# MarcinKadziolka/nerf-sampling

Hardware: NVIDIA B200
Metric: rays_per_sec (higher is better)
Workload: dtype fp16 operands, fp32 accumulate (+ bf16 hi/lo split re-evaluation of the guard band)

## Files before the change

nerf_sampling_b200/csrc/mlp_fast.cuh:

```cuda
#pragma once
#include <type_traits>

#include "ptx.cuh"

namespace b200 {
namespace fast {

constexpr int TILE_M = 128;
constexpr int KC_STRIDE = 2048;
constexpr int ENC_KB = 16;
constexpr int VIEW_KB = 20;
constexpr int TILE_KC = 44;
constexpr int TILE_ACT_BYTES = TILE_KC * KC_STRIDE;
constexpr int RING_BYTES = 32768;
constexpr int AUX_FLOATS = 3080;
constexpr int SF32_FLOATS = 1032;
constexpr int SBIAS16 = 7 * 256;
constexpr int THREADS = 512;
constexpr int NSTEPS = 9;
constexpr int EPI_WARP0 = 4, EPI_WARPS = 8, PRO_WARP0 = 12, PRO_WARPS = 4;
constexpr size_t FOLD_BIAS_OFF = 65 * 16384;
constexpr size_t WPACK_BYTES = FOLD_BIAS_OFF + 512;

enum : uint32_t { AUX_B0 = 0, AUX_BF = 2048, AUX_BV = 2304, AUX_WA = 2432, AUX_BA = 2688, AUX_WR = 2692, AUX_BR = 3076 };
enum : uint32_t { SF_B7 = 0, SF_BV = 256, SF_WA = 384, SF_BA = 640, SF_WR = 644, SF_BR = 1028 };

__host__ __device__ constexpr int step_nk1(int s) { return s == 0 ? 4 : 16; }
__host__ __device__ constexpr int step_kb1(int s) { return s == 0 ? ENC_KB : 0; }
__host__ __device__ constexpr int step_nk2(int s) { return s == 5 ? 4 : (s == NSTEPS - 1 ? 2 : 0); }
__host__ __device__ constexpr int step_kb2(int s) { return s == 5 ? ENC_KB : VIEW_KB; }
__host__ __device__ constexpr int step_n(int s) { return s == NSTEPS - 1 ? 128 : 256; }
__host__ __device__ constexpr int step_nk(int s) { return step_nk1(s) + step_nk2(s); }
__host__ __device__ constexpr int step_stages(int s) { return s == NSTEPS - 1 ? 5 : step_nk(s) / 2; }
__host__ __device__ constexpr uint32_t step_woff(int s) {
  uint32_t o = 0;
  for (int i = 0; i < s; ++i) o += static_cast<uint32_t>(step_stages(i)) * 16384u;
  return o;
}

struct alignas(64) TMap {
  uint8_t bytes[128];
};

struct FastParams {
  const uint8_t* wpack;
  const float* aux;
  int n_rows;
  int S;
  const float* rays_o;
  const float* rays_d;
  const float* viewdirs;
  const float* z;
  const float* pts;
  float* out;
  int* guard_count;
  int* guard_list;
  int guard_cap;
  float guard_kappa;
  long long* timeline;
};

#ifdef B200NERF_TIMELINE
#define TL_STAMP(role, idx, j)                                                                         \
  do {                                                                                                 \
    if (p.timeline != nullptr && blockIdx.x == 0 && (idx) < 80) p.timeline[((role) * 80 + (idx)) * 4 + (j)] = clock64(); \
  } while (0)
#else
#define TL_STAMP(role, idx, j) \
  do {                         \
  } while (0)
#endif

constexpr int NSTAGE = 4;
constexpr int STAGE_BYTES = RING_BYTES / NSTAGE;
constexpr int NCTA = 2;
#ifndef B200NERF_FAST_STAGGER
#define B200NERF_FAST_STAGGER 5
#endif
constexpr int STAGGER = B200NERF_FAST_STAGGER;

struct __align__(16) Tail {
  uint64_t full[NSTAGE];
  uint64_t empty[NSTAGE];
  uint64_t acc_full[2];
  uint64_t a_ready[2];
  uint64_t enc_ready[2];
  uint64_t view_ready[2];
  uint64_t pts_free[2];
  uint64_t view_free[2];
  uint32_t tmem_base;
  uint32_t pad[3];
  float alpha_part[2][TILE_M];
  float eabs_part[2][TILE_M];
  float rgb_part[2][3][TILE_M];
};

__host__ __device__ constexpr int smem_bytes() {
  return 2 * TILE_ACT_BYTES + RING_BYTES + SF32_FLOATS * 4 + SBIAS16 * 2 + static_cast<int>(sizeof(Tail));
}

template <bool FP16>
__device__ __forceinline__ void store8(uint8_t* dst, const float (&v)[8]) {
  *reinterpret_cast<uint4*>(dst) = make_uint4(pack_half2<FP16, false>(v[0], v[1]), pack_half2<FP16, false>(v[2], v[3]),
                                              pack_half2<FP16, false>(v[4], v[5]), pack_half2<FP16, false>(v[6], v[7]));
}

template <bool FP16, int NF, int NCHUNK>
__device__ __forceinline__ void encode_store(const float (&x)[3], uint8_t* dst ) {
  float sn[NF][3], cs[NF][3];
#pragma unroll
  for (int t = 0; t < 3; ++t) {
    sincosf(x[t], &sn[0][t], &cs[0][t]);
    if (NF > 5) sincosf(x[t] * 32.0f, &sn[5][t], &cs[5][t]);
#pragma unroll
    for (int j = 1; j < NF; ++j) {
      if (j == 5) continue;
      const float s = sn[j - 1][t], c = cs[j - 1][t];
      sn[j][t] = 2.0f * s * c;
      cs[j][t] = (c - s) * (c + s);
    }
  }
  constexpr int NCOL = 3 + 6 * NF;
#pragma unroll
  for (int ch = 0; ch < NCHUNK; ++ch) {
    float v[8];
#pragma unroll
    for (int i = 0; i < 8; ++i) {
      const int cc = ch * 8 + i;
      if (cc < 3) v[i] = x[cc];
      else if (cc < NCOL) v[i] = ((cc - 3) % 6) < 3 ? sn[(cc - 3) / 6][(cc - 3) % 6] : cs[(cc - 3) / 6][(cc - 3) % 6 - 3];
      else v[i] = 0.f;
    }
    store8<FP16>(dst + ch * KC_STRIDE, v);
  }
}

template <bool FP16>
__device__ __noinline__ void encode_pts_lt10(int nf, float x0, float x1, float x2, uint8_t* dst) {
  const float x[3] = {x0, x1, x2};
  switch (nf) {
    case 1: encode_store<FP16, 1, 8>(x, dst); break;
    case 2: encode_store<FP16, 2, 8>(x, dst); break;
    case 3: encode_store<FP16, 3, 8>(x, dst); break;
    case 4: encode_store<FP16, 4, 8>(x, dst); break;
    case 5: encode_store<FP16, 5, 8>(x, dst); break;
    case 6: encode_store<FP16, 6, 8>(x, dst); break;
    case 7: encode_store<FP16, 7, 8>(x, dst); break;
    case 8: encode_store<FP16, 8, 8>(x, dst); break;
    default: encode_store<FP16, 9, 8>(x, dst); break;
  }
}
template <bool FP16>
__device__ __noinline__ void encode_view_lt4(int nv, float v0, float v1, float v2, uint8_t* dst) {
  const float v[3] = {v0, v1, v2};
  switch (nv) {
    case 1: encode_store<FP16, 1, 4>(v, dst); break;
    case 2: encode_store<FP16, 2, 4>(v, dst); break;
    default: encode_store<FP16, 3, 4>(v, dst); break;
  }
}
// ... 71 lines not shown
  epi_store32_packed<RELU, FP16>(va, bias16 + 64, dst + 8 * KC_STRIDE);
  tmem_ld_wait();
  epi_store32_packed<RELU, FP16>(vb, bias16 + 96, dst + 12 * KC_STRIDE);
}

template <int MODE, bool FP16>
__device__ __forceinline__ void epilogue_store(uint32_t tacc, const float* bias, const float* hw, uint8_t* dst,
                                               float& hsum, float& habs) {
  uint32_t va[32], vb[32];
  tmem_ld_32x32b_x32(tacc, va);
  tmem_ld_wait();
  tmem_ld_32x32b_x32(tacc + 32, vb);
  epi_store32<MODE, FP16>(va, bias, hw, dst, hsum, habs);
  tmem_ld_wait();
  tmem_ld_32x32b_x32(tacc + 64, va);
  epi_store32<MODE, FP16>(vb, bias + 32, hw + 32, dst + 4 * KC_STRIDE, hsum, habs);
  tmem_ld_wait();
  tmem_ld_32x32b_x32(tacc + 96, vb);
  epi_store32<MODE, FP16>(va, bias + 64, hw + 64, dst + 8 * KC_STRIDE, hsum, habs);
  tmem_ld_wait();
  epi_store32<MODE, FP16>(vb, bias + 96, hw + 96, dst + 12 * KC_STRIDE, hsum, habs);
}

__device__ __forceinline__ void epi_rgb32(const uint32_t (&v)[32], const float* bias, const float* wr, float& r, float& g,
                                          float& b) {
#pragma unroll
  for (int j = 0; j < 32; j += 4) {
    const float4 bb = *reinterpret_cast<const float4*>(bias + j);
    const float4 w0 = *reinterpret_cast<const float4*>(wr + j);
    const float4 w1 = *reinterpret_cast<const float4*>(wr + 128 + j);
    const float4 w2 = *reinterpret_cast<const float4*>(wr + 256 + j);
    const float x0 = fmaxf(__uint_as_float(v[j]) + bb.x, 0.f), x1 = fmaxf(__uint_as_float(v[j + 1]) + bb.y, 0.f);
    const float x2 = fmaxf(__uint_as_float(v[j + 2]) + bb.z, 0.f), x3 = fmaxf(__uint_as_float(v[j + 3]) + bb.w, 0.f);
    r = fmaf(x0, w0.x, r); r = fmaf(x1, w0.y, r); r = fmaf(x2, w0.z, r); r = fmaf(x3, w0.w, r);
    g = fmaf(x0, w1.x, g); g = fmaf(x1, w1.y, g); g = fmaf(x2, w1.z, g); g = fmaf(x3, w1.w, g);
    b = fmaf(x0, w2.x, b); b = fmaf(x1, w2.y, b); b = fmaf(x2, w2.z, b); b = fmaf(x3, w2.w, b);
  }
}

__device__ __forceinline__ bool input_is_finite(const FastParams& p, int grow) {
  const int ray = grow / p.S;
  float m = 0.f;
  if (p.pts != nullptr) {
#pragma unroll
    for (int t = 0; t < 3; ++t) m += fabsf(__ldg(p.pts + static_cast<size_t>(grow) * 3 + t));
  } else {
    const float zz = __ldg(p.z + grow);
#pragma unroll
    for (int t = 0; t < 3; ++t) m += fabsf(__fadd_rn(__ldg(p.rays_o + ray * 3 + t), __fmul_rn(__ldg(p.rays_d + ray * 3 + t), zz)));
  }
#pragma unroll
  for (int t = 0; t < 3; ++t) m += fabsf(__ldg(p.viewdirs + ray * 3 + t));
  return m < __int_as_float(0x7f800000);
}

template <bool FP16>
__global__ void __launch_bounds__(THREADS, 1)
nerf_fast_kernel(const __grid_constant__ FastParams p, const __grid_constant__ TMap tm_full) {
  extern __shared__ __align__(1024) uint8_t smem[];
  uint8_t* act = smem;
  uint8_t* ring = smem + 2 * TILE_ACT_BYTES;
  float* sf32 = reinterpret_cast<float*>(ring + RING_BYTES);
  uint16_t* sb16 = reinterpret_cast<uint16_t*>(ring + RING_BYTES + SF32_FLOATS * 4);
  Tail* tail = reinterpret_cast<Tail*>(ring + RING_BYTES + SF32_FLOATS * 4 + SBIAS16 * 2);

  const int warp = __shfl_sync(0xffffffffu, static_cast<int>(threadIdx.x >> 5), 0);
  const int lane = threadIdx.x & 31;
  const uint32_t rank = __shfl_sync(0xffffffffu, cluster_ctarank(), 0);
  const bool leader = rank == 0;
  const int cluster_id = blockIdx.x / NCTA;
  const int n_clusters = gridDim.x / NCTA;
  const int num_tiles = (p.n_rows + TILE_M - 1) / TILE_M;
  const int n_units = (num_tiles + 2 * NCTA - 1) / (2 * NCTA);
  const int my_units = cluster_id < n_units ? (n_units - cluster_id + n_clusters - 1) / n_clusters : 0;
  const int n_ticks = my_units > 0 ? my_units * NSTEPS + STAGGER : 0;

  if (threadIdx.x == 0) {
    for (int i = 0; i < NSTAGE; ++i) {
      mbar_init(&tail->full[i], 1);
      mbar_init(&tail->empty[i], 1);
    }
    for (int i = 0; i < 2; ++i) {
      mbar_init(&tail->acc_full[i], 1);
      mbar_init(&tail->a_ready[i], EPI_WARPS * NCTA);
      mbar_init(&tail->enc_ready[i], PRO_WARPS * NCTA);
      mbar_init(&tail->view_ready[i], PRO_WARPS * NCTA);
      mbar_init(&tail->pts_free[i], 1);
      mbar_init(&tail->view_free[i], 1);
    }
    fence_mbar_init();
  }
  if (warp == 2) {
    tmem_alloc_cg2(&tail->tmem_base, 512);
    tmem_relinquish_cg2();
  }
  for (int i = threadIdx.x; i < SF32_FLOATS; i += THREADS) {
    if (i >= 256 && i < 384) {
      sf32[i] = reinterpret_cast<const float*>(p.wpack + FOLD_BIAS_OFF)[i - 256];
    } else {
      const uint32_t src = i < 256 ? AUX_B0 + 7 * 256 + i : i < 640 ? AUX_WA + (i - 384)
                         : i < 644 ? AUX_BA + (i - 640) : i < 1028 ? AUX_WR + (i - 644) : AUX_BR + (i - 1028);
      sf32[i] = p.aux[src];
    }
  }
  for (int i = threadIdx.x; i < SBIAS16; i += THREADS) {
    sb16[i] = static_cast<uint16_t>(pack_half2<FP16, false>(p.aux[AUX_B0 + i], 0.f) & 0xffffu);
  }
  tc_fence_before();
  cluster_sync_all();
  tc_fence_after();
  const uint32_t tmem_base = __shfl_sync(0xffffffffu, tail->tmem_base, 0);
  const uint32_t tail_addr = smem_u32(tail);
  const uint32_t full_addr = tail_addr + offsetof(Tail, full), empty_addr = tail_addr + offsetof(Tail, empty);

  if (warp == 0) {
    if (lane == 0) tma_prefetch_desc(&tm_full);
    const uint32_t ring_addr = smem_u32(ring);
    const uint32_t lead_full = mapa_u32(full_addr, 0);
    uint32_t stage = 0, phase = 0;
    for (int i = 0; i < n_ticks; ++i) {
      for (int slot = 0; slot < 2; ++slot) {
        const int j = i - slot * STAGGER;
        if (j < 0 || j >= my_units * NSTEPS) continue;
        const int s = j % NSTEPS;
        const int n2 = step_stages(s);
        const int row0 = static_cast<int>((step_woff(s) + rank * static_cast<uint32_t>(n2) * STAGE_BYTES) / 512u);
        for (int k2 = 0; k2 < n2; ++k2) {
          mbar_wait_sleepy(empty_addr + stage * 8u, phase ^ 1u, 100);
          if (elect_one()) {
            if (leader) mbar_arrive_expect_tx_addr(full_addr + stage * 8u, 2u * STAGE_BYTES);
            tma_load_2d_cg2(ring_addr + stage * STAGE_BYTES, &tm_full, 0, row0 + k2 * (STAGE_BYTES / 512), lead_full + stage * 8u);
          }
          __syncwarp();
          if (++stage == NSTAGE) {
            stage = 0;
            phase ^= 1u;
          }
        }
      }
    }
  } else if (warp == 1) {
    if (leader) {
      const uint32_t act_addr = smem_u32(act);
      const uint32_t ring_addr = smem_u32(ring);
      const uint32_t acc_full_addr = tail_addr + offsetof(Tail, acc_full);
      const uint32_t a_ready_addr = tail_addr + offsetof(Tail, a_ready);
      const uint32_t enc_ready_addr = tail_addr + offsetof(Tail, enc_ready);
      const uint32_t view_ready_addr = tail_addr + offsetof(Tail, view_ready);
      const uint32_t pts_free_addr = tail_addr + offsetof(Tail, pts_free);
      const uint32_t view_free_addr = tail_addr + offsetof(Tail, view_free);
      constexpr uint32_t A_STEP = (2 * KC_STRIDE) >> 4;
      constexpr uint32_t DESC_HI = static_cast<uint32_t>(((128ull >> 4) << 32 | (1ull << 46)) >> 32);
      constexpr uint32_t A_LBO = (KC_STRIDE >> 4) << 16;
      uint32_t stage = 0, phase = 0, ca[2] = {0, 0}, ce[2] = {0, 0}, cv[2] = {0, 0};

      auto issue_stage = [&](auto acc_first, uint32_t d_tmem, uint32_t a_lo, uint32_t b_lbo, uint32_t piece16, uint32_t idesc) {
        mbar_wait_lean(full_addr + stage * 8u, phase);
        tc_fence_after();
        const uint32_t b_lo = b_lbo | ((ring_addr + stage * STAGE_BYTES) >> 4);
        if (elect_one()) {
          const uint64_t a0 = (static_cast<uint64_t>(DESC_HI) << 32) | a_lo;
          const uint64_t b0 = (static_cast<uint64_t>(DESC_HI) << 32) | b_lo;
          tc_mma_f16_cg2_imm<decltype(acc_first)::value>(d_tmem, a0, b0, idesc);
          tc_mma_f16_cg2_imm<true>(d_tmem, a0 + A_STEP, b0 + piece16, idesc);
          tc_commit_cg2_addr(empty_addr + stage * 8u, 3);
        }
        stage = (stage + 1) & (NSTAGE - 1);
        phase ^= (stage == 0);
      };

      auto issue_stage4 = [&](auto acc_first, auto two_only, uint32_t d_tmem, uint32_t a_lo, uint32_t a_lo2, uint32_t idesc) {
        constexpr uint32_t B_LBO = ((128u * 8u) >> 4) << 16, PIECE16 = 128;
        mbar_wait_lean(full_addr + stage * 8u, phase);
        tc_fence_after();
        const uint32_t b_lo = B_LBO | ((ring_addr + stage * STAGE_BYTES) >> 4);
        if (elect_one()) {
          const uint64_t a0 = (static_cast<uint64_t>(DESC_HI) << 32) | a_lo;
          const uint64_t a2 = (static_cast<uint64_t>(DESC_HI) << 32) | a_lo2;
          const uint64_t b0 = (static_cast<uint64_t>(DESC_HI) << 32) | b_lo;
          tc_mma_f16_cg2_imm<decltype(acc_first)::value>(d_tmem, a0, b0, idesc);
          tc_mma_f16_cg2_imm<true>(d_tmem, a0 + A_STEP, b0 + PIECE16, idesc);
          if (!decltype(two_only)::value) {
            tc_mma_f16_cg2_imm<true>(d_tmem, a2, b0 + 2 * PIECE16, idesc);
            tc_mma_f16_cg2_imm<true>(d_tmem, a2 + A_STEP, b0 + 3 * PIECE16, idesc);
          }
          tc_commit_cg2_addr(empty_addr + stage * 8u, 3);
        }
        stage = (stage + 1) & (NSTAGE - 1);
        phase ^= (stage == 0);
      };

#pragma unroll 1
      for (int i = 0; i < n_ticks; ++i) {
#pragma unroll
        for (int slot = 0; slot < 2; ++slot) {
          const int j = i - slot * STAGGER;
          if (j < 0 || j >= my_units * NSTEPS) continue;
          const int s = j % NSTEPS;
          const bool first = j < NSTEPS;
          const int n1 = step_nk1(s) / 2, n2 = step_nk(s) / 2;
          const uint32_t n = static_cast<uint32_t>(step_n(s));
          const uint32_t piece16 = n;
          const uint32_t idesc = umma_idesc_f16(FP16 ? 0u : 1u, 256, n);
          const uint32_t b_lbo = ((n * 8u) >> 4) << 16;
          const uint32_t kb1 = step_kb1(s), kb2 = step_kb2(s);
          [[maybe_unused]] const int tl_idx = j * 2 + slot;
          if (lane == 0) TL_STAMP(0, tl_idx, 0);
          if (s == 0) {
            mbar_wait_lean(enc_ready_addr + slot * 8u, ce[slot]++ & 1u);
            if (!first) mbar_wait_lean(a_ready_addr + slot * 8u, ca[slot]++ & 1u);
          } else {
            mbar_wait_lean(a_ready_addr + slot * 8u, ca[slot]++ & 1u);
          }
          if (s == NSTEPS - 1) mbar_wait_lean(view_ready_addr + slot * 8u, cv[slot]++ & 1u);
          if (lane == 0) TL_STAMP(0, tl_idx, 1);
          const uint32_t d_tmem = tmem_base + slot * 256u;
          const uint32_t a_base = A_LBO | ((act_addr + slot * TILE_ACT_BYTES) >> 4);
          uint32_t a_lo = a_base + kb1 * A_STEP;
          if (s == NSTEPS - 1) {
            issue_stage4(std::false_type{}, std::false_type{}, d_tmem, a_lo, a_lo + 2 * A_STEP, idesc);
#pragma unroll 1
            for (int k4 = 1; k4 < 4; ++k4) {
              a_lo += 4 * A_STEP;
              issue_stage4(std::true_type{}, std::false_type{}, d_tmem, a_lo, a_lo + 2 * A_STEP, idesc);
            }
            a_lo = a_base + VIEW_KB * A_STEP;
            issue_stage4(std::true_type{}, std::true_type{}, d_tmem, a_lo, a_lo, idesc);
          } else {
            issue_stage(std::false_type{}, d_tmem, a_lo, b_lbo, piece16, idesc);
            for (int k2 = 1; k2 < n1; ++k2) {
              a_lo += 2 * A_STEP;
              issue_stage(std::true_type{}, d_tmem, a_lo, b_lbo, piece16, idesc);
            }
            a_lo = a_base + kb2 * A_STEP;
            for (int k2 = n1; k2 < n2; ++k2) {
              issue_stage(std::true_type{}, d_tmem, a_lo, b_lbo, piece16, idesc);
              a_lo += 2 * A_STEP;
            }
          }
          if (elect_one()) {
            tc_commit_cg2_addr(acc_full_addr + slot * 8u, 3);
            if (s == 5) tc_commit_cg2_addr(pts_free_addr + slot * 8u, 3);
            if (s == NSTEPS - 1) tc_commit_cg2_addr(view_free_addr + slot * 8u, 3);
          }
          if (lane == 0) TL_STAMP(0, tl_idx, 2);
        }
      }
    }
  } else if (warp >= PRO_WARP0) {
    const int row = (warp - PRO_WARP0) * 32 + lane;
    const int row_off = (row >> 3) * 128 + (row & 7) * 16;
    const uint32_t pts_free_addr = tail_addr + offsetof(Tail, pts_free);
    const uint32_t view_free_addr = tail_addr + offsetof(Tail, view_free);
    const uint32_t enc_bar = mapa_u32(tail_addr + offsetof(Tail, enc_ready), 0);
    const uint32_t view_bar = mapa_u32(tail_addr + offsetof(Tail, view_ready), 0);
    const int nf = static_cast<int>(sf32[SF_BA + 1]), nv = static_cast<int>(sf32[SF_BA + 2]);
    const bool nf_full = nf == 0 || nf == 10, nv_full = nv == 0 || nv == 4;
    uint32_t cp[2] = {0, 0}, cw[2] = {0, 0};
    bool first = true;
    for (int u = cluster_id; u < n_units; u += n_clusters) {
#pragma unroll
      for (int slot = 0; slot < 2; ++slot) {
        const int grow = ((u * NCTA + static_cast<int>(rank)) * 2 + slot) * TILE_M + row;
        float x[3] = {0.f, 0.f, 0.f};
        if (grow < p.n_rows) {
          if (p.pts != nullptr) {
#pragma unroll
            for (int t = 0; t < 3; ++t) x[t] = __ldg(p.pts + static_cast<size_t>(grow) * 3 + t);
          } else {
            const int ray = grow / p.S;
            const float zz = __ldg(p.z + grow);
#pragma unroll
            for (int t = 0; t < 3; ++t)
              x[t] = __fadd_rn(__ldg(p.rays_o + ray * 3 + t), __fmul_rn(__ldg(p.rays_d + ray * 3 + t), zz));
          }
        }
        if (!first) {
          mbar_wait_sleepy(pts_free_addr + slot * 8u, cp[slot]++ & 1u, 500);
          tc_fence_after();
        }
        uint8_t* enc_dst = act + slot * TILE_ACT_BYTES + ENC_KB * 2 * KC_STRIDE + row_off;
        if (nf_full) encode_store<FP16, 10, 8>(x, enc_dst);
        else encode_pts_lt10<FP16>(nf, x[0], x[1], x[2], enc_dst);
        fence_proxy_async_smem();
        __syncwarp();
        if (lane == 0) mbar_arrive_remote(enc_bar + slot * 8u);
        float v[3] = {0.f, 0.f, 0.f};
        if (grow < p.n_rows) {
          const int ray = grow / p.S;
#pragma unroll
          for (int t = 0; t < 3; ++t) v[t] = __ldg(p.viewdirs + ray * 3 + t);
        }
        if (!first) {
          mbar_wait_sleepy(view_free_addr + slot * 8u, cw[slot]++ & 1u, 500);
          tc_fence_after();
        }
        uint8_t* view_dst = act + slot * TILE_ACT_BYTES + VIEW_KB * 2 * KC_STRIDE + row_off;
        if (nv_full) encode_store<FP16, 4, 4>(v, view_dst);
        else encode_view_lt4<FP16>(nv, v[0], v[1], v[2], view_dst);
        fence_proxy_async_smem();
        __syncwarp();
        if (lane == 0) mbar_arrive_remote(view_bar + slot * 8u);
      }
      first = false;
    }
  } else if (warp >= EPI_WARP0) {
    const int q = warp & 3;
    const int hf = (warp - EPI_WARP0) >> 2;
    const int row = q * 32 + lane;
    const int row_off = (row >> 3) * 128 + (row & 7) * 16;
    const uint32_t t_lane = tmem_base + (static_cast<uint32_t>(q * 32) << 16);
    const uint32_t acc_full_addr = tail_addr + offsetof(Tail, acc_full);
    const uint32_t rdy_bar = mapa_u32(tail_addr + offsetof(Tail, a_ready), 0);
    uint32_t cf[2] = {0, 0};
    float alpha_keep[2] = {0.f, 0.f}, eabs_keep[2] = {0.f, 0.f};

#pragma unroll 1
    for (int i = 0; i < n_ticks; ++i) {
      {
#pragma unroll
        for (int slot = 0; slot < 2; ++slot) {
          const int j = i - slot * STAGGER;
          if (j < 0 || j >= my_units * NSTEPS) continue;
          const int s = j % NSTEPS;
          const int u = cluster_id + (j / NSTEPS) * n_clusters;
          [[maybe_unused]] const int tl_idx = j * 2 + slot;
          if (lane == 0 && q == 0) TL_STAMP(1 + hf, tl_idx, 0);
          mbar_wait_lean(acc_full_addr + slot * 8u, cf[slot]++ & 1u);
          tc_fence_after();
          if (lane == 0 && q == 0) TL_STAMP(1 + hf, tl_idx, 1);
          const uint32_t tacc = t_lane + slot * 256u;
          uint8_t* a_tile = act + slot * TILE_ACT_BYTES;
          if (s < NSTEPS - 1) {
            uint8_t* dst = a_tile + hf * 16 * KC_STRIDE + row_off;
            if (s == 7) {
              float hs = 0.f, ha = 0.f;
              const int grow0 = ((u * NCTA + static_cast<int>(rank)) * 2 + slot) * TILE_M + (row & ~31);
              const bool need_abs = p.guard_count != nullptr && (p.S - 1 - grow0 % p.S) < 32;
              if (need_abs) epilogue_store<1, FP16>(tacc + hf * 128, sf32 + SF_B7 + hf * 128, sf32 + SF_WA + hf * 128, dst, hs, ha);
              else epilogue_store<3, FP16>(tacc + hf * 128, sf32 + SF_B7 + hf * 128, sf32 + SF_WA + hf * 128, dst, hs, ha);
              if (hf == 1) {
                tail->alpha_part[slot][row] = hs;
                tail->eabs_part[slot][row] = ha;
              } else {
                alpha_keep[slot] = hs;
                eabs_keep[slot] = ha;
              }
            } else {
              epilogue_store_packed<true, FP16>(tacc + hf * 128, sb16 + s * 256 + hf * 128, dst);
            }
          } else {
            float r = 0.f, g = 0.f, b = 0.f;
            uint32_t va[32], vb[32];
            tmem_ld_32x32b_x32(tacc + hf * 64, va);
            tmem_ld_wait();
            tmem_ld_32x32b_x32(tacc + hf * 64 + 32, vb);
            epi_rgb32(va, sf32 + SF_BV + hf * 64, sf32 + SF_WR + hf * 64, r, g, b);
            tmem_ld_wait();
            epi_rgb32(vb, sf32 + SF_BV + hf * 64 + 32, sf32 + SF_WR + hf * 64 + 32, r, g, b);
            if (hf == 1) {
              tail->rgb_part[slot][0][row] = r;
              tail->rgb_part[slot][1][row] = g;
              tail->rgb_part[slot][2][row] = b;
            }
            named_bar_sync(2 + q, 64);
            if (hf == 0) {
              r += tail->rgb_part[slot][0][row];
              g += tail->rgb_part[slot][1][row];
              b += tail->rgb_part[slot][2][row];
              const int grow = ((u * NCTA + static_cast<int>(rank)) * 2 + slot) * TILE_M + row;
              const bool valid = grow < p.n_rows;
              float sigma = alpha_keep[slot] + tail->alpha_part[slot][row] + sf32[SF_BA];
              if (valid) {
                if (!input_is_finite(p, grow)) r = g = b = sigma = __int_as_float(0x7fc00000);
                reinterpret_cast<float4*>(p.out)[grow] =
                    make_float4(r + sf32[SF_BR], g + sf32[SF_BR + 1], b + sf32[SF_BR + 2], sigma);
              }
              if (p.guard_count != nullptr) {
                const float eabs = eabs_keep[slot] + tail->eabs_part[slot][row] + fabsf(sf32[SF_BA]);
                const bool flag = valid && (grow % p.S) == p.S - 1 && !(fabsf(sigma) >= p.guard_kappa * eabs);
                const uint32_t m = __ballot_sync(0xffffffffu, flag);
                if (m != 0) {
                  int base = 0;
                  if (lane == 0) base = atomicAdd(p.guard_count, __popc(m));
                  base = __shfl_sync(0xffffffffu, base, 0);
                  const int idx = base + __popc(m & ((1u << lane) - 1u));
                  if (flag && idx < p.guard_cap) p.guard_list[idx] = grow;
                }
              }
            }
          }
          if (s < NSTEPS - 1) fence_proxy_async_smem();
          tc_fence_before();
          __syncwarp();
          if (lane == 0) mbar_arrive_remote(rdy_bar + slot * 8u);
          if (lane == 0 && q == 0) TL_STAMP(1 + hf, tl_idx, 2);
        }
      }
    }
  }

  __syncwarp();
  tc_fence_before();
  cluster_sync_all();
  if (warp == 2) tmem_dealloc_cg2(tmem_base, 512);
}

}
}
```

nerf_sampling_b200/csrc/ptx.cuh:

```cuda
#pragma once
#include <cstdint>
#include <cuda_runtime.h>

namespace b200 {

__device__ __forceinline__ uint32_t smem_u32(const void* p) {
  return static_cast<uint32_t>(__cvta_generic_to_shared(p));
}

__device__ __forceinline__ void mbar_init(uint64_t* bar, uint32_t count) {
  asm volatile("mbarrier.init.shared::cta.b64 [%0], %1;" ::"r"(smem_u32(bar)), "r"(count) : "memory");
}
__device__ __forceinline__ void fence_mbar_init() {
  asm volatile("fence.mbarrier_init.release.cluster;" ::: "memory");
}
__device__ __forceinline__ void mbar_arrive(uint64_t* bar) {
  asm volatile("mbarrier.arrive.shared::cta.b64 _, [%0];" ::"r"(smem_u32(bar)) : "memory");
}
__device__ __forceinline__ void mbar_arrive_expect_tx(uint64_t* bar, uint32_t bytes) {
  asm volatile("mbarrier.arrive.expect_tx.shared::cta.b64 _, [%0], %1;" ::"r"(smem_u32(bar)), "r"(bytes)
               : "memory");
}
__device__ __forceinline__ bool mbar_try_wait(uint64_t* bar, uint32_t parity) {
  uint32_t ok;
// ... 201 lines not shown
  uint32_t polls = 0;
  for (;;) {
    uint32_t ok;
    asm volatile(
        "{\n\t"
        ".reg .pred p;\n\t"
        "mbarrier.try_wait.parity.shared::cta.b64 p, [%1], %2;\n\t"
        "selp.u32 %0, 1, 0, p;\n\t"
        "}\n"
        : "=r"(ok)
        : "r"(bar_addr), "r"(parity)
        : "memory");
    if (ok) return;
    if (++polls > (1u << 24)) {
      printf("b200nerf: mbarrier wait timed out (block %d thread %d bar %u parity %u)\n", blockIdx.x, threadIdx.x, bar_addr, parity);
      __trap();
    }
  }
}
__device__ __forceinline__ void mbar_wait_sleepy(uint32_t bar_addr, uint32_t parity, uint32_t ns) {
  uint32_t polls = 0;
  for (;;) {
    uint32_t ok;
    asm volatile(
        "{\n\t"
        ".reg .pred p;\n\t"
        "mbarrier.try_wait.parity.shared::cta.b64 p, [%1], %2;\n\t"
        "selp.u32 %0, 1, 0, p;\n\t"
        "}\n"
        : "=r"(ok)
        : "r"(bar_addr), "r"(parity)
        : "memory");
    if (ok) return;
    __nanosleep(ns);
    if (++polls > (1u << 24)) {
      printf("b200nerf: mbarrier wait timed out (block %d thread %d bar %u parity %u)\n", blockIdx.x, threadIdx.x, bar_addr, parity);
      __trap();
    }
  }
}

__device__ __forceinline__ void mbar_arrive_remote(uint32_t cluster_addr) {
  asm volatile("mbarrier.arrive.shared::cluster.b64 _, [%0];" ::"r"(cluster_addr) : "memory");
}
__device__ __forceinline__ void mbar_arrive_expect_tx_addr(uint32_t bar_addr, uint32_t bytes) {
  asm volatile("mbarrier.arrive.expect_tx.shared::cta.b64 _, [%0], %1;" ::"r"(bar_addr), "r"(bytes) : "memory");
}
__device__ __forceinline__ bool elect_one() {
  uint32_t pred;
  asm volatile(
      "{\n\t"
      ".reg .pred p;\n\t"
      "elect.sync _|p, 0xffffffff;\n\t"
      "selp.u32 %0, 1, 0, p;\n\t"
      "}\n"
      : "=r"(pred));
  return pred != 0;
}
__device__ __forceinline__ void tc_commit_cg2_addr(uint32_t bar_addr, uint16_t cta_mask) {
  asm volatile("tcgen05.commit.cta_group::2.mbarrier::arrive::one.shared::cluster.multicast::cluster.b64 [%0], %1;" ::"r"(bar_addr),
               "h"(cta_mask)
               : "memory");
}
template <bool ACC>
__device__ __forceinline__ void tc_mma_f16_cg2_imm(uint32_t d_tmem, uint64_t a_desc, uint64_t b_desc, uint32_t idesc) {
  if (ACC) {
    asm volatile(
        "{\n\t.reg .pred p;\n\tsetp.eq.u32 p, 1, 1;\n\t"
        "tcgen05.mma.cta_group::2.kind::f16 [%0], %1, %2, %3, p;\n\t}\n" ::"r"(d_tmem),
        "l"(a_desc), "l"(b_desc), "r"(idesc)
        : "memory");
  } else {
    asm volatile(
        "{\n\t.reg .pred p;\n\tsetp.eq.u32 p, 1, 0;\n\t"
        "tcgen05.mma.cta_group::2.kind::f16 [%0], %1, %2, %3, p;\n\t}\n" ::"r"(d_tmem),
        "l"(a_desc), "l"(b_desc), "r"(idesc)
        : "memory");
  }
}

__device__ __forceinline__ void named_bar_sync(uint32_t id, uint32_t nthreads) {
  asm volatile("bar.sync %0, %1;" ::"r"(id), "r"(nthreads) : "memory");
}
__device__ __forceinline__ uint32_t pack_bf16x2(float lo_elem, float hi_elem) {
  uint32_t r;
  asm("cvt.rn.bf16x2.f32 %0, %1, %2;" : "=r"(r) : "f"(hi_elem), "f"(lo_elem));
  return r;
}

}
```

Measured before the change: 17.89 million.

## Give each accumulator slot its own epilogue warpgroup and rebalance registers with setmaxnreg

Raises the block from 512 to 768 threads so each of the two TMEM accumulator slots gets a dedicated set of 8 epilogue warps, instead of one set of epilogue warps alternating between both slots. This is meant to remove serialization between the two slots' epilogues so the MMA issuer waits less on a_ready. Control warps release registers via setmaxnreg.dec and worker warps claim more via setmaxnreg.inc, and the slot stagger is bumped from 5 to 6. The cost is lower per-thread register headroom, which risks spills, plus more warps contending for issue slots and shared memory.

```diff
diff --git a/nerf_sampling_b200/csrc/mlp_fast.cuh b/nerf_sampling_b200/csrc/mlp_fast.cuh
--- a/nerf_sampling_b200/csrc/mlp_fast.cuh
+++ b/nerf_sampling_b200/csrc/mlp_fast.cuh
@@ -16,9 +16,11 @@
 constexpr int AUX_FLOATS = 3080;
 constexpr int SF32_FLOATS = 1032;
 constexpr int SBIAS16 = 7 * 256;
-constexpr int THREADS = 512;
+constexpr int THREADS = 768;
 constexpr int NSTEPS = 9;
-constexpr int EPI_WARP0 = 4, EPI_WARPS = 8, PRO_WARP0 = 12, PRO_WARPS = 4;
+constexpr int EPI_WARP0 = 4, EPI_WARPS_PER_SLOT = 8, PRO_WARP0 = 20, PRO_WARPS = 4;
+constexpr int REG_CTRL = 40, REG_WORK = 88;
+static_assert(REG_CTRL + 5 * REG_WORK <= 6 * 80, "setmaxnreg budgets exceed the launch allocation");
 constexpr size_t FOLD_BIAS_OFF = 65 * 16384;
 constexpr size_t WPACK_BYTES = FOLD_BIAS_OFF + 512;
 
@@ -75,7 +77,7 @@
 constexpr int STAGE_BYTES = RING_BYTES / NSTAGE;
 constexpr int NCTA = 2;
 #ifndef B200NERF_FAST_STAGGER
-#define B200NERF_FAST_STAGGER 5
+#define B200NERF_FAST_STAGGER 6
 #endif
 constexpr int STAGGER = B200NERF_FAST_STAGGER;
 
@@ -313,7 +315,7 @@
     }
     for (int i = 0; i < 2; ++i) {
       mbar_init(&tail->acc_full[i], 1);
-      mbar_init(&tail->a_ready[i], EPI_WARPS * NCTA);
+      mbar_init(&tail->a_ready[i], EPI_WARPS_PER_SLOT * NCTA);
       mbar_init(&tail->enc_ready[i], PRO_WARPS * NCTA);
       mbar_init(&tail->view_ready[i], PRO_WARPS * NCTA);
       mbar_init(&tail->pts_free[i], 1);
@@ -344,141 +346,145 @@
   const uint32_t tail_addr = smem_u32(tail);
   const uint32_t full_addr = tail_addr + offsetof(Tail, full), empty_addr = tail_addr + offsetof(Tail, empty);
 
-  if (warp == 0) {
-    if (lane == 0) tma_prefetch_desc(&tm_full);
-    const uint32_t ring_addr = smem_u32(ring);
-    const uint32_t lead_full = mapa_u32(full_addr, 0);
-    uint32_t stage = 0, phase = 0;
-    for (int i = 0; i < n_ticks; ++i) {
-      for (int slot = 0; slot < 2; ++slot) {
-        const int j = i - slot * STAGGER;
-        if (j < 0 || j >= my_units * NSTEPS) continue;
-        const int s = j % NSTEPS;
-        const int n2 = step_stages(s);
-        const int row0 = static_cast<int>((step_woff(s) + rank * static_cast<uint32_t>(n2) * STAGE_BYTES) / 512u);
-        for (int k2 = 0; k2 < n2; ++k2) {
-          mbar_wait_sleepy(empty_addr + stage * 8u, phase ^ 1u, 100);
-          if (elect_one()) {
-            if (leader) mbar_arrive_expect_tx_addr(full_addr + stage * 8u, 2u * STAGE_BYTES);
-            tma_load_2d_cg2(ring_addr + stage * STAGE_BYTES, &tm_full, 0, row0 + k2 * (STAGE_BYTES / 512), lead_full + stage * 8u);
-          }
-          __syncwarp();
-          if (++stage == NSTAGE) {
-            stage = 0;
-            phase ^= 1u;
-          }
-        }
-      }
-    }
-  } else if (warp == 1) {
-    if (leader) {
-      const uint32_t act_addr = smem_u32(act);
+  if (warp < EPI_WARP0) {
+    setmaxnreg_dec<REG_CTRL>();
+    if (warp == 0) {
+      if (lane == 0) tma_prefetch_desc(&tm_full);
       const uint32_t ring_addr = smem_u32(ring);
-      const uint32_t acc_full_addr = tail_addr + offsetof(Tail, acc_full);
-      const uint32_t a_ready_addr = tail_addr + offsetof(Tail, a_ready);
-      const uint32_t enc_ready_addr = tail_addr + offsetof(Tail, enc_ready);
-      const uint32_t view_ready_addr = tail_addr + offsetof(Tail, view_ready);
-      const uint32_t pts_free_addr = tail_addr + offsetof(Tail, pts_free);
-      const uint32_t view_free_addr = tail_addr + offsetof(Tail, view_free);
-      constexpr uint32_t A_STEP = (2 * KC_STRIDE) >> 4;
-      constexpr uint32_t DESC_HI = static_cast<uint32_t>(((128ull >> 4) << 32 | (1ull << 46)) >> 32);
-      constexpr uint32_t A_LBO = (KC_STRIDE >> 4) << 16;
-      uint32_t stage = 0, phase = 0, ca[2] = {0, 0}, ce[2] = {0, 0}, cv[2] = {0, 0};
-
-      auto issue_stage = [&](auto acc_first, uint32_t d_tmem, uint32_t a_lo, uint32_t b_lbo, uint32_t piece16, uint32_t idesc) {
-        mbar_wait_lean(full_addr + stage * 8u, phase);
-        tc_fence_after();
-        const uint32_t b_lo = b_lbo | ((ring_addr + stage * STAGE_BYTES) >> 4);
-        if (elect_one()) {
-          const uint64_t a0 = (static_cast<uint64_t>(DESC_HI) << 32) | a_lo;
-          const uint64_t b0 = (static_cast<uint64_t>(DESC_HI) << 32) | b_lo;
-          tc_mma_f16_cg2_imm<decltype(acc_first)::value>(d_tmem, a0, b0, idesc);
-          tc_mma_f16_cg2_imm<true>(d_tmem, a0 + A_STEP, b0 + piece16, idesc);
-          tc_commit_cg2_addr(empty_addr + stage * 8u, 3);
-        }
-        stage = (stage + 1) & (NSTAGE - 1);
-        phase ^= (stage == 0);
-      };
-
-      auto issue_stage4 = [&](auto acc_first, auto two_only, uint32_t d_tmem, uint32_t a_lo, uint32_t a_lo2, uint32_t idesc) {
-        constexpr uint32_t B_LBO = ((128u * 8u) >> 4) << 16, PIECE16 = 128;
-        mbar_wait_lean(full_addr + stage * 8u, phase);
-        tc_fence_after();
-        const uint32_t b_lo = B_LBO | ((ring_addr + stage * STAGE_BYTES) >> 4);
-        if (elect_one()) {
-          const uint64_t a0 = (static_cast<uint64_t>(DESC_HI) << 32) | a_lo;
-          const uint64_t a2 = (static_cast<uint64_t>(DESC_HI) << 32) | a_lo2;
-          const uint64_t b0 = (static_cast<uint64_t>(DESC_HI) << 32) | b_lo;
-          tc_mma_f16_cg2_imm<decltype(acc_first)::value>(d_tmem, a0, b0, idesc);
-          tc_mma_f16_cg2_imm<true>(d_tmem, a0 + A_STEP, b0 + PIECE16, idesc);
-          if (!decltype(two_only)::value) {
-            tc_mma_f16_cg2_imm<true>(d_tmem, a2, b0 + 2 * PIECE16, idesc);
-            tc_mma_f16_cg2_imm<true>(d_tmem, a2 + A_STEP, b0 + 3 * PIECE16, idesc);
-          }
-          tc_commit_cg2_addr(empty_addr + stage * 8u, 3);
-        }
-        stage = (stage + 1) & (NSTAGE - 1);
-        phase ^= (stage == 0);
-      };
-
-#pragma unroll 1
+      const uint32_t lead_full = mapa_u32(full_addr, 0);
+      uint32_t stage = 0, phase = 0;
       for (int i = 0; i < n_ticks; ++i) {
-#pragma unroll
         for (int slot = 0; slot < 2; ++slot) {
           const int j = i - slot * STAGGER;
           if (j < 0 || j >= my_units * NSTEPS) continue;
           const int s = j % NSTEPS;
-          const bool first = j < NSTEPS;
-          const int n1 = step_nk1(s) / 2, n2 = step_nk(s) / 2;
-          const uint32_t n = static_cast<uint32_t>(step_n(s));
-          const uint32_t piece16 = n;
-          const uint32_t idesc = umma_idesc_f16(FP16 ? 0u : 1u, 256, n);
-          const uint32_t b_lbo = ((n * 8u) >> 4) << 16;
-          const uint32_t kb1 = step_kb1(s), kb2 = step_kb2(s);
-          [[maybe_unused]] const int tl_idx = j * 2 + slot;
-          if (lane == 0) TL_STAMP(0, tl_idx, 0);
-          if (s == 0) {
-            mbar_wait_lean(enc_ready_addr + slot * 8u, ce[slot]++ & 1u);
-            if (!first) mbar_wait_lean(a_ready_addr + slot * 8u, ca[slot]++ & 1u);
-          } else {
-            mbar_wait_lean(a_ready_addr + slot * 8u, ca[slot]++ & 1u);
-          }
-          if (s == NSTEPS - 1) mbar_wait_lean(view_ready_addr + slot * 8u, cv[slot]++ & 1u);
-          if (lane == 0) TL_STAMP(0, tl_idx, 1);
-          const uint32_t d_tmem = tmem_base + slot * 256u;
-          const uint32_t a_base = A_LBO | ((act_addr + slot * TILE_ACT_BYTES) >> 4);
-          uint32_t a_lo = a_base + kb1 * A_STEP;
-          if (s == NSTEPS - 1) {
-            issue_stage4(std::false_type{}, std::false_type{}, d_tmem, a_lo, a_lo + 2 * A_STEP, idesc);
+          const int n2 = step_stages(s);
+          const int row0 = static_cast<int>((step_woff(s) + rank * static_cast<uint32_t>(n2) * STAGE_BYTES) / 512u);
+          for (int k2 = 0; k2 < n2; ++k2) {
+            mbar_wait_sleepy(empty_addr + stage * 8u, phase ^ 1u, 100);
+            if (elect_one()) {
+              if (leader) mbar_arrive_expect_tx_addr(full_addr + stage * 8u, 2u * STAGE_BYTES);
+              tma_load_2d_cg2(ring_addr + stage * STAGE_BYTES, &tm_full, 0, row0 + k2 * (STAGE_BYTES / 512), lead_full + stage * 8u);
+            }
+            __syncwarp();
+            if (++stage == NSTAGE) {
+              stage = 0;
+              phase ^= 1u;
+            }
+          }
+        }
+      }
+    } else if (warp == 1) {
+      if (leader) {
+        const uint32_t act_addr = smem_u32(act);
+        const uint32_t ring_addr = smem_u32(ring);
+        const uint32_t acc_full_addr = tail_addr + offsetof(Tail, acc_full);
+        const uint32_t a_ready_addr = tail_addr + offsetof(Tail, a_ready);
+        const uint32_t enc_ready_addr = tail_addr + offsetof(Tail, enc_ready);
+        const uint32_t view_ready_addr = tail_addr + offsetof(Tail, view_ready);
+        const uint32_t pts_free_addr = tail_addr + offsetof(Tail, pts_free);
+        const uint32_t view_free_addr = tail_addr + offsetof(Tail, view_free);
+        constexpr uint32_t A_STEP = (2 * KC_STRIDE) >> 4;
+        constexpr uint32_t DESC_HI = static_cast<uint32_t>(((128ull >> 4) << 32 | (1ull << 46)) >> 32);
+        constexpr uint32_t A_LBO = (KC_STRIDE >> 4) << 16;
+        uint32_t stage = 0, phase = 0, ca[2] = {0, 0}, ce[2] = {0, 0}, cv[2] = {0, 0};
+
+        auto issue_stage = [&](auto acc_first, uint32_t d_tmem, uint32_t a_lo, uint32_t b_lbo, uint32_t piece16, uint32_t idesc) {
+          mbar_wait_lean(full_addr + stage * 8u, phase);
+          tc_fence_after();
+          const uint32_t b_lo = b_lbo | ((ring_addr + stage * STAGE_BYTES) >> 4);
+          if (elect_one()) {
+            const uint64_t a0 = (static_cast<uint64_t>(DESC_HI) << 32) | a_lo;
+            const uint64_t b0 = (static_cast<uint64_t>(DESC_HI) << 32) | b_lo;
+            tc_mma_f16_cg2_imm<decltype(acc_first)::value>(d_tmem, a0, b0, idesc);
+            tc_mma_f16_cg2_imm<true>(d_tmem, a0 + A_STEP, b0 + piece16, idesc);
+            tc_commit_cg2_addr(empty_addr + stage * 8u, 3);
+          }
+          stage = (stage + 1) & (NSTAGE - 1);
+          phase ^= (stage == 0);
+        };
+
+        auto issue_stage4 = [&](auto acc_first, auto two_only, uint32_t d_tmem, uint32_t a_lo, uint32_t a_lo2, uint32_t idesc) {
+          constexpr uint32_t B_LBO = ((128u * 8u) >> 4) << 16, PIECE16 = 128;
+          mbar_wait_lean(full_addr + stage * 8u, phase);
+          tc_fence_after();
+          const uint32_t b_lo = B_LBO | ((ring_addr + stage * STAGE_BYTES) >> 4);
+          if (elect_one()) {
+            const uint64_t a0 = (static_cast<uint64_t>(DESC_HI) << 32) | a_lo;
+            const uint64_t a2 = (static_cast<uint64_t>(DESC_HI) << 32) | a_lo2;
+            const uint64_t b0 = (static_cast<uint64_t>(DESC_HI) << 32) | b_lo;
+            tc_mma_f16_cg2_imm<decltype(acc_first)::value>(d_tmem, a0, b0, idesc);
+            tc_mma_f16_cg2_imm<true>(d_tmem, a0 + A_STEP, b0 + PIECE16, idesc);
+            if (!decltype(two_only)::value) {
+              tc_mma_f16_cg2_imm<true>(d_tmem, a2, b0 + 2 * PIECE16, idesc);
+              tc_mma_f16_cg2_imm<true>(d_tmem, a2 + A_STEP, b0 + 3 * PIECE16, idesc);
+            }
+            tc_commit_cg2_addr(empty_addr + stage * 8u, 3);
+          }
+          stage = (stage + 1) & (NSTAGE - 1);
+          phase ^= (stage == 0);
+        };
+
 #pragma unroll 1
-            for (int k4 = 1; k4 < 4; ++k4) {
-              a_lo += 4 * A_STEP;
-              issue_stage4(std::true_type{}, std::false_type{}, d_tmem, a_lo, a_lo + 2 * A_STEP, idesc);
+        for (int i = 0; i < n_ticks; ++i) {
+#pragma unroll
+          for (int slot = 0; slot < 2; ++slot) {
+            const int j = i - slot * STAGGER;
+            if (j < 0 || j >= my_units * NSTEPS) continue;
+            const int s = j % NSTEPS;
+            const bool first = j < NSTEPS;
+            const int n1 = step_nk1(s) / 2, n2 = step_nk(s) / 2;
+            const uint32_t n = static_cast<uint32_t>(step_n(s));
+            const uint32_t piece16 = n;
+            const uint32_t idesc = umma_idesc_f16(FP16 ? 0u : 1u, 256, n);
+            const uint32_t b_lbo = ((n * 8u) >> 4) << 16;
+            const uint32_t kb1 = step_kb1(s), kb2 = step_kb2(s);
+            [[maybe_unused]] const int tl_idx = j * 2 + slot;
+            if (lane == 0) TL_STAMP(0, tl_idx, 0);
+            if (s == 0) {
+              mbar_wait_lean(enc_ready_addr + slot * 8u, ce[slot]++ & 1u);
+              if (!first) mbar_wait_lean(a_ready_addr + slot * 8u, ca[slot]++ & 1u);
+            } else {
+              mbar_wait_lean(a_ready_addr + slot * 8u, ca[slot]++ & 1u);
             }
-            a_lo = a_base + VIEW_KB * A_STEP;
-            issue_stage4(std::true_type{}, std::true_type{}, d_tmem, a_lo, a_lo, idesc);
-          } else {
-            issue_stage(std::false_type{}, d_tmem, a_lo, b_lbo, piece16, idesc);
-            for (int k2 = 1; k2 < n1; ++k2) {
-              a_lo += 2 * A_STEP;
-              issue_stage(std::true_type{}, d_tmem, a_lo, b_lbo, piece16, idesc);
+            if (s == NSTEPS - 1) mbar_wait_lean(view_ready_addr + slot * 8u, cv[slot]++ & 1u);
+            if (lane == 0) TL_STAMP(0, tl_idx, 1);
+            const uint32_t d_tmem = tmem_base + slot * 256u;
+            const uint32_t a_base = A_LBO | ((act_addr + slot * TILE_ACT_BYTES) >> 4);
+            uint32_t a_lo = a_base + kb1 * A_STEP;
+            if (s == NSTEPS - 1) {
+              issue_stage4(std::false_type{}, std::false_type{}, d_tmem, a_lo, a_lo + 2 * A_STEP, idesc);
+#pragma unroll 1
+              for (int k4 = 1; k4 < 4; ++k4) {
+                a_lo += 4 * A_STEP;
+                issue_stage4(std::true_type{}, std::false_type{}, d_tmem, a_lo, a_lo + 2 * A_STEP, idesc);
+              }
+              a_lo = a_base + VIEW_KB * A_STEP;
+              issue_stage4(std::true_type{}, std::true_type{}, d_tmem, a_lo, a_lo, idesc);
+            } else {
+              issue_stage(std::false_type{}, d_tmem, a_lo, b_lbo, piece16, idesc);
+              for (int k2 = 1; k2 < n1; ++k2) {
+                a_lo += 2 * A_STEP;
+                issue_stage(std::true_type{}, d_tmem, a_lo, b_lbo, piece16, idesc);
+              }
+              a_lo = a_base + kb2 * A_STEP;
+              for (int k2 = n1; k2 < n2; ++k2) {
+                issue_stage(std::true_type{}, d_tmem, a_lo, b_lbo, piece16, idesc);
+                a_lo += 2 * A_STEP;
+              }
             }
-            a_lo = a_base + kb2 * A_STEP;
-            for (int k2 = n1; k2 < n2; ++k2) {
-              issue_stage(std::true_type{}, d_tmem, a_lo, b_lbo, piece16, idesc);
-              a_lo += 2 * A_STEP;
+            if (elect_one()) {
+              tc_commit_cg2_addr(acc_full_addr + slot * 8u, 3);
+              if (s == 5) tc_commit_cg2_addr(pts_free_addr + slot * 8u, 3);
+              if (s == NSTEPS - 1) tc_commit_cg2_addr(view_free_addr + slot * 8u, 3);
             }
-          }
-          if (elect_one()) {
-            tc_commit_cg2_addr(acc_full_addr + slot * 8u, 3);
-            if (s == 5) tc_commit_cg2_addr(pts_free_addr + slot * 8u, 3);
-            if (s == NSTEPS - 1) tc_commit_cg2_addr(view_free_addr + slot * 8u, 3);
-          }
-          if (lane == 0) TL_STAMP(0, tl_idx, 2);
+            if (lane == 0) TL_STAMP(0, tl_idx, 2);
+          }
         }
       }
     }
   } else if (warp >= PRO_WARP0) {
+    setmaxnreg_inc<REG_WORK>();
     const int row = (warp - PRO_WARP0) * 32 + lane;
     const int row_off = (row >> 3) * 128 + (row & 7) * 16;
     const uint32_t pts_free_addr = tail_addr + offsetof(Tail, pts_free);
@@ -535,99 +541,94 @@
       }
       first = false;
     }
-  } else if (warp >= EPI_WARP0) {
+  } else {
+    setmaxnreg_inc<REG_WORK>();
     const int q = warp & 3;
-    const int hf = (warp - EPI_WARP0) >> 2;
+    const int slot = (warp - EPI_WARP0) / EPI_WARPS_PER_SLOT;
+    const int hf = ((warp - EPI_WARP0) >> 2) & 1;
     const int row = q * 32 + lane;
     const int row_off = (row >> 3) * 128 + (row & 7) * 16;
     const uint32_t t_lane = tmem_base + (static_cast<uint32_t>(q * 32) << 16);
     const uint32_t acc_full_addr = tail_addr + offsetof(Tail, acc_full);
     const uint32_t rdy_bar = mapa_u32(tail_addr + offsetof(Tail, a_ready), 0);
-    uint32_t cf[2] = {0, 0};
-    float alpha_keep[2] = {0.f, 0.f}, eabs_keep[2] = {0.f, 0.f};
+    uint32_t cf = 0;
+    float alpha_keep = 0.f, eabs_keep = 0.f;
 
 #pragma unroll 1
-    for (int i = 0; i < n_ticks; ++i) {
-      {
-#pragma unroll
-        for (int slot = 0; slot < 2; ++slot) {
-          const int j = i - slot * STAGGER;
-          if (j < 0 || j >= my_units * NSTEPS) continue;
-          const int s = j % NSTEPS;
-          const int u = cluster_id + (j / NSTEPS) * n_clusters;
-          [[maybe_unused]] const int tl_idx = j * 2 + slot;
-          if (lane == 0 && q == 0) TL_STAMP(1 + hf, tl_idx, 0);
-          mbar_wait_lean(acc_full_addr + slot * 8u, cf[slot]++ & 1u);
-          tc_fence_after();
-          if (lane == 0 && q == 0) TL_STAMP(1 + hf, tl_idx, 1);
-          const uint32_t tacc = t_lane + slot * 256u;
-          uint8_t* a_tile = act + slot * TILE_ACT_BYTES;
-          if (s < NSTEPS - 1) {
-            uint8_t* dst = a_tile + hf * 16 * KC_STRIDE + row_off;
-            if (s == 7) {
-              float hs = 0.f, ha = 0.f;
-              const int grow0 = ((u * NCTA + static_cast<int>(rank)) * 2 + slot) * TILE_M + (row & ~31);
-              const bool need_abs = p.guard_count != nullptr && (p.S - 1 - grow0 % p.S) < 32;
-              if (need_abs) epilogue_store<1, FP16>(tacc + hf * 128, sf32 + SF_B7 + hf * 128, sf32 + SF_WA + hf * 128, dst, hs, ha);
-              else epilogue_store<3, FP16>(tacc + hf * 128, sf32 + SF_B7 + hf * 128, sf32 + SF_WA + hf * 128, dst, hs, ha);
-              if (hf == 1) {
-                tail->alpha_part[slot][row] = hs;
-                tail->eabs_part[slot][row] = ha;
-              } else {
-                alpha_keep[slot] = hs;
-                eabs_keep[slot] = ha;
-              }
-            } else {
-              epilogue_store_packed<true, FP16>(tacc + hf * 128, sb16 + s * 256 + hf * 128, dst);
+    for (int j = 0; j < my_units * NSTEPS; ++j) {
+      const int s = j % NSTEPS;
+      const int u = cluster_id + (j / NSTEPS) * n_clusters;
+      [[maybe_unused]] const int tl_idx = j * 2 + slot;
+      if (lane == 0 && q == 0) TL_STAMP(1 + hf, tl_idx, 0);
+      mbar_wait_lean(acc_full_addr + slot * 8u, cf++ & 1u);
+      tc_fence_after();
+      if (lane == 0 && q == 0) TL_STAMP(1 + hf, tl_idx, 1);
+      const uint32_t tacc = t_lane + slot * 256u;
+      uint8_t* a_tile = act + slot * TILE_ACT_BYTES;
+      if (s < NSTEPS - 1) {
+        uint8_t* dst = a_tile + hf * 16 * KC_STRIDE + row_off;
+        if (s == 7) {
+          float hs = 0.f, ha = 0.f;
+          const int grow0 = ((u * NCTA + static_cast<int>(rank)) * 2 + slot) * TILE_M + (row & ~31);
+          const bool need_abs = p.guard_count != nullptr && (p.S - 1 - grow0 % p.S) < 32;
+          if (need_abs) epilogue_store<1, FP16>(tacc + hf * 128, sf32 + SF_B7 + hf * 128, sf32 + SF_WA + hf * 128, dst, hs, ha);
+          else epilogue_store<3, FP16>(tacc + hf * 128, sf32 + SF_B7 + hf * 128, sf32 + SF_WA + hf * 128, dst, hs, ha);
+          if (hf == 1) {
+            tail->alpha_part[slot][row] = hs;
+            tail->eabs_part[slot][row] = ha;
+          } else {
+            alpha_keep = hs;
+            eabs_keep = ha;
+          }
+        } else {
+          epilogue_store_packed<true, FP16>(tacc + hf * 128, sb16 + s * 256 + hf * 128, dst);
+        }
+      } else {
+        float r = 0.f, g = 0.f, b = 0.f;
+        uint32_t va[32], vb[32];
+        tmem_ld_32x32b_x32(tacc + hf * 64, va);
+        tmem_ld_wait();
+        tmem_ld_32x32b_x32(tacc + hf * 64 + 32, vb);
+        epi_rgb32(va, sf32 + SF_BV + hf * 64, sf32 + SF_WR + hf * 64, r, g, b);
+        tmem_ld_wait();
+        epi_rgb32(vb, sf32 + SF_BV + hf * 64 + 32, sf32 + SF_WR + hf * 64 + 32, r, g, b);
+        if (hf == 1) {
+          tail->rgb_part[slot][0][row] = r;
+          tail->rgb_part[slot][1][row] = g;
+          tail->rgb_part[slot][2][row] = b;
+        }
+        named_bar_sync(2 + 4 * slot + q, 64);
+        if (hf == 0) {
+          r += tail->rgb_part[slot][0][row];
+          g += tail->rgb_part[slot][1][row];
+          b += tail->rgb_part[slot][2][row];
+          const int grow = ((u * NCTA + static_cast<int>(rank)) * 2 + slot) * TILE_M + row;
+          const bool valid = grow < p.n_rows;
+          float sigma = alpha_keep + tail->alpha_part[slot][row] + sf32[SF_BA];
+          if (valid) {
+            if (!input_is_finite(p, grow)) r = g = b = sigma = __int_as_float(0x7fc00000);
+            reinterpret_cast<float4*>(p.out)[grow] =
+                make_float4(r + sf32[SF_BR], g + sf32[SF_BR + 1], b + sf32[SF_BR + 2], sigma);
+          }
+          if (p.guard_count != nullptr) {
+            const float eabs = eabs_keep + tail->eabs_part[slot][row] + fabsf(sf32[SF_BA]);
+            const bool flag = valid && (grow % p.S) == p.S - 1 && !(fabsf(sigma) >= p.guard_kappa * eabs);
+            const uint32_t m = __ballot_sync(0xffffffffu, flag);
+            if (m != 0) {
+              int base = 0;
+              if (lane == 0) base = atomicAdd(p.guard_count, __popc(m));
+              base = __shfl_sync(0xffffffffu, base, 0);
+              const int idx = base + __popc(m & ((1u << lane) - 1u));
+              if (flag && idx < p.guard_cap) p.guard_list[idx] = grow;
             }
-          } else {
-            float r = 0.f, g = 0.f, b = 0.f;
-            uint32_t va[32], vb[32];
-            tmem_ld_32x32b_x32(tacc + hf * 64, va);
-            tmem_ld_wait();
-            tmem_ld_32x32b_x32(tacc + hf * 64 + 32, vb);
-            epi_rgb32(va, sf32 + SF_BV + hf * 64, sf32 + SF_WR + hf * 64, r, g, b);
-            tmem_ld_wait();
-            epi_rgb32(vb, sf32 + SF_BV + hf * 64 + 32, sf32 + SF_WR + hf * 64 + 32, r, g, b);
-            if (hf == 1) {
-              tail->rgb_part[slot][0][row] = r;
-              tail->rgb_part[slot][1][row] = g;
-              tail->rgb_part[slot][2][row] = b;
-            }
-            named_bar_sync(2 + q, 64);
-            if (hf == 0) {
-              r += tail->rgb_part[slot][0][row];
-              g += tail->rgb_part[slot][1][row];
-              b += tail->rgb_part[slot][2][row];
-              const int grow = ((u * NCTA + static_cast<int>(rank)) * 2 + slot) * TILE_M + row;
-              const bool valid = grow < p.n_rows;
-              float sigma = alpha_keep[slot] + tail->alpha_part[slot][row] + sf32[SF_BA];
-              if (valid) {
-                if (!input_is_finite(p, grow)) r = g = b = sigma = __int_as_float(0x7fc00000);
-                reinterpret_cast<float4*>(p.out)[grow] =
-                    make_float4(r + sf32[SF_BR], g + sf32[SF_BR + 1], b + sf32[SF_BR + 2], sigma);
-              }
-              if (p.guard_count != nullptr) {
-                const float eabs = eabs_keep[slot] + tail->eabs_part[slot][row] + fabsf(sf32[SF_BA]);
-                const bool flag = valid && (grow % p.S) == p.S - 1 && !(fabsf(sigma) >= p.guard_kappa * eabs);
-                const uint32_t m = __ballot_sync(0xffffffffu, flag);
-                if (m != 0) {
-                  int base = 0;
-                  if (lane == 0) base = atomicAdd(p.guard_count, __popc(m));
-                  base = __shfl_sync(0xffffffffu, base, 0);
-                  const int idx = base + __popc(m & ((1u << lane) - 1u));
-                  if (flag && idx < p.guard_cap) p.guard_list[idx] = grow;
-                }
-              }
-            }
-          }
-          if (s < NSTEPS - 1) fence_proxy_async_smem();
-          tc_fence_before();
-          __syncwarp();
-          if (lane == 0) mbar_arrive_remote(rdy_bar + slot * 8u);
-          if (lane == 0 && q == 0) TL_STAMP(1 + hf, tl_idx, 2);
+          }
         }
       }
+      if (s < NSTEPS - 1) fence_proxy_async_smem();
+      tc_fence_before();
+      __syncwarp();
+      if (lane == 0) mbar_arrive_remote(rdy_bar + slot * 8u);
+      if (lane == 0 && q == 0) TL_STAMP(1 + hf, tl_idx, 2);
     }
   }
 
diff --git a/nerf_sampling_b200/csrc/ptx.cuh b/nerf_sampling_b200/csrc/ptx.cuh
--- a/nerf_sampling_b200/csrc/ptx.cuh
+++ b/nerf_sampling_b200/csrc/ptx.cuh
@@ -307,6 +307,10 @@
 __device__ __forceinline__ void named_bar_sync(uint32_t id, uint32_t nthreads) {
   asm volatile("bar.sync %0, %1;" ::"r"(id), "r"(nthreads) : "memory");
 }
+template <int N>
+__device__ __forceinline__ void setmaxnreg_dec() { asm volatile("setmaxnreg.dec.sync.aligned.u32 %0;" ::"n"(N)); }
+template <int N>
+__device__ __forceinline__ void setmaxnreg_inc() { asm volatile("setmaxnreg.inc.sync.aligned.u32 %0;" ::"n"(N)); }
 __device__ __forceinline__ uint32_t pack_bf16x2(float lo_elem, float hi_elem) {
   uint32_t r;
   asm("cvt.rn.bf16x2.f32 %0, %1, %2;" : "=r"(r) : "f"(hi_elem), "f"(lo_elem));
```

After: 18.10 million (median of 6 runs). 1.2% higher.
